# iesl/anncur

Measured on AMD Instinct MI355X. Metric: queries/sec + Top-k-Recall@100 vs exact, CUR-256 on QxI score matrix, higher is better.
Workload: dtype bf16; 1 GPU; cfg2: Q=10000/GPU x I=100000 bf16 score matrix, 256 anchor items, 512 anchor queries, k=100, k_retvr=100; step = gather C_q + fused S_hat/top-k + exact top-k scan + overlap/recall; Q_per_gpu=10000, I=100000, anchors=256, anchor_queries=512, k=100, k_retvr=100

## Files before the change

### anncur_amd/csrc/score16.hpp

```cpp
#pragma once

typedef __attribute__((ext_vector_type(4))) float f32x4;

template <int KP, int NW = 4>
struct Fused16Cfg {
	static constexpr int WAVES = NW;
	static constexpr int KS32 = KP / 32;
	static constexpr int K = KP / 16;
	static constexpr int CPR = KP / 8;
	static constexpr int TILE_BYTES = TILE_I * KP * 2;
	static constexpr int QCAP = 1024;
	static constexpr int DRAIN_AT = 192;
	static constexpr int QUEUE_OFF = 2 * TILE_BYTES;
	static constexpr int CNT_OFF = QUEUE_OFF + NW * QCAP * 8;
	static constexpr int TICKET_OFF = CNT_OFF + NW * 64 * 4;
	static constexpr int PIECES = TILE_BYTES / 1024 / NW;
	static_assert(PIECES >= 1, "a tile holds at least one 1 KB piece per wave");
	static constexpr int LVL_OFF = TICKET_OFF + 16;
	static constexpr int LCNT_OFF = LVL_OFF + NW * 64 * 4 * LADDER_LEVELS;
	static constexpr int JCUR_OFF = LCNT_OFF + NW * 64 * 16;
	static constexpr int LDS_BYTES = JCUR_OFF + NW * 64 * 4;
	static_assert(NW != 4 || LDS_BYTES <= 80 * 1024, "two workgroups per CU");
	static_assert(LADDER_LEVELS == 8, "two 128-bit reads per query; eight 16-bit fields in four counter words");
	static constexpr int BQ = 64 * NW;
};
#ifndef ANNCUR_LADDER_PERIOD
#define ANNCUR_LADDER_PERIOD 16
#endif
constexpr int LADDER_PERIOD = ANNCUR_LADDER_PERIOD;
constexpr uint32_t WQ_ITEM_BITS = 26, WQ_ITEM_MASK = (1u << WQ_ITEM_BITS) - 1u;

struct WaveQueue {
	uint32_t base, limit;
	uint32_t cnt;
	uint2 *seg;
	uint32_t q_stride8;
	uint32_t capg, n_items;
	int lane;
	uint32_t lad_on, lvl, jcur;
	uint32_t *lcnt;
};

template <bool LAD = false>
__device__ __forceinline__ void wq_drain(const WaveQueue &w, uint32_t &fill) {
	const uint32_t n = (fill - w.base) >> 3;
	unsigned char *const segb = reinterpret_cast<unsigned char *>(w.seg);
#pragma nounroll
	for (uint32_t i0 = 0; i0 < n; i0 += 64) {
		const uint32_t i = i0 + (uint32_t)w.lane;
		if (i < n) {
			const uint2 e = lds_load_u64(w.base + i * 8u);
			const uint32_t item = e.y & WQ_ITEM_MASK, ql = e.y >> WQ_ITEM_BITS;
			if (item < w.n_items) {
				uint32_t pos = 0;
#if defined(__HIP_DEVICE_COMPILE__)
				const uint32_t one = 1u;
				asm volatile("ds_add_rtn_u32 %0, %1, %2\n\ts_waitcnt lgkmcnt(0)" : "=&v"(pos) : "v"(w.cnt + ql * 4u), "v"(one) : "memory");
#endif
				if (pos < w.capg) *reinterpret_cast<uint2 *>(segb + (ql * w.q_stride8 + pos * 8u)) = make_uint2(e.x, item);
				if (LAD && w.lad_on) {
					f32x4 la = {0.f, 0.f, 0.f, 0.f}, lb = {0.f, 0.f, 0.f, 0.f};
					uint32_t jc = 0;
#if defined(__HIP_DEVICE_COMPILE__)
					asm volatile("ds_read_b128 %0, %3\n\tds_read_b128 %1, %3 offset:16\n\tds_read_b32 %2, %4\n\ts_waitcnt lgkmcnt(0)"
								 : "=&v"(la), "=&v"(lb), "=&v"(jc) : "v"(w.lvl + ql * 32u), "v"(w.jcur + ql * 4u) : "memory");
#endif
					const float v = __uint_as_float(e.x);
					const uint32_t j = (uint32_t)(v >= la[0]) + (uint32_t)(v >= la[1]) + (uint32_t)(v >= la[2]) + (uint32_t)(v >= la[3])
									   + (uint32_t)(v >= lb[0]) + (uint32_t)(v >= lb[1]) + (uint32_t)(v >= lb[2]) + (uint32_t)(v >= lb[3]);
					if (j > jc)
						(void)__hip_atomic_fetch_add(w.lcnt + ql * 4u + ((j - 1u) >> 1), 1u << (16u * ((j - 1u) & 1u)), __ATOMIC_RELAXED, __HIP_MEMORY_SCOPE_AGENT);
				}
			}
		}
	}
	fill = w.base;
}

__device__ __forceinline__ void filter16_one(float v, uint32_t code, float tau, uint32_t item0c, const WaveQueue &w, uint32_t &fill) {
	const bool hit = v >= tau;
	const unsigned long long m = __ballot(hit);
	if (__builtin_expect(m != 0ull, 0)) {
		if (hit) {
			const uint32_t rank = __builtin_amdgcn_mbcnt_hi((uint32_t)(m >> 32), __builtin_amdgcn_mbcnt_lo((uint32_t)m, 0u));
			lds_write_2x32(fill + rank * 8u, __float_as_uint(v), item0c + code);
		}
		fill += 8u * (uint32_t)__builtin_popcountll(m);
	}
}

__device__ __forceinline__ uint32_t opaque_u32(uint32_t x) {
#if defined(__HIP_DEVICE_COMPILE__)
	asm volatile("" : "+v"(x));
#endif
	return x;
}
__device__ __forceinline__ void ladder_fetch(const uint32_t *lcnt_wave, uint32_t land, int lane) {
#if defined(__HIP_DEVICE_COMPILE__)
	const uint32_t voff = (uint32_t)lane * 16u;
	asm volatile("s_mov_b32 m0, %0\n\ts_nop 0\n\tglobal_load_lds_dwordx4 %1, %2 sc1" ::"s"(land), "v"(voff), "s"(lcnt_wave) : "memory", "m0");
#endif
}

__device__ __forceinline__ void ladder_refresh(uint32_t lcnt_lane, uint32_t lvl_lane, uint32_t jcur_lane, uint32_t k, int c16, float (&tau)[4]) {
	u32x4 c = {0u, 0u, 0u, 0u};
	f32x4 la = {0.f, 0.f, 0.f, 0.f}, lb = {0.f, 0.f, 0.f, 0.f};
	uint32_t jc = 0;
#if defined(__HIP_DEVICE_COMPILE__)
	asm volatile("ds_read_b128 %0, %4\n\tds_read_b128 %1, %5\n\tds_read_b128 %2, %5 offset:16\n\tds_read_b32 %3, %6\n\ts_waitcnt lgkmcnt(0)"
				 : "=&v"(c), "=&v"(la), "=&v"(lb), "=&v"(jc) : "v"(lcnt_lane), "v"(lvl_lane), "v"(jcur_lane) : "memory");
#endif
	const float lv[8] = {la[0], la[1], la[2], la[3], lb[0], lb[1], lb[2], lb[3]};
	uint32_t cum = 0, jn = 0;
	float tn = -INFINITY;
#pragma unroll
	for (int j = 8; j >= 1; --j) {
		cum += (c[(j - 1) >> 1] >> (16 * ((j - 1) & 1))) & 0xffffu;
		const bool take = jn == 0u && cum >= k;
		jn = take ? (uint32_t)j : jn;
		tn = take ? lv[j - 1] : tn;
	}
	if (jn > jc) lds_write_u32(jcur_lane, jn);
#pragma unroll
	for (int t = 0; t < 4; ++t) {
		const float o = __int_as_float(__builtin_amdgcn_ds_bpermute((16 * t + c16) * 4, __float_as_int(tn)));
		tau[t] = fmaxf(tau[t], o);
	}
}

template <int KP, int CUR>
__device__ __forceinline__ void stagger16_tile(const uint32_t (&aoff)[Fused16Cfg<KP>::K], const bf16x8 (&xb)[4][Fused16Cfg<KP>::KS32], f32x4 (&accP)[2][2],
												const float (&tau)[4], const float (&tau_prev)[2], uint32_t item0, uint32_t item0_prev, const WaveQueue &w,
												uint32_t &fill) {
	using C = Fused16Cfg<KP>;
	constexpr int K = C::K, AR = 5, DIST = 3, OFF = CUR * C::TILE_BYTES;
	constexpr int EPS = 16 / K > 0 ? 16 / K : 1;
	static_assert(K <= 16 && 2 * K >= DIST, "staggered path: 4..16 steps per half");
	u32x4 ring[AR];
#pragma unroll
	for (int i = 0; i < DIST; ++i) lds_read_frag<OFF>(ring[i], aoff[i % K]);
	f32x4 accA[2][2], accB[2][2];
#pragma unroll
	for (int ih = 0; ih < 2; ++ih)
#pragma unroll
		for (int q = 0; q < 2; ++q) { accA[ih][q] = (f32x4){0.f, 0.f, 0.f, 0.f}; accB[ih][q] = (f32x4){0.f, 0.f, 0.f, 0.f}; }
#define F16_ELEM(ACC, e, QS0, TAU, ITEM0)                                                                                       \
	filter16_one(ACC[(e) >> 3][((e) >> 2) & 1][(e) & 3],                                                                        \
				 (uint32_t)((((e) >> 3) * 16 + ((e) & 3)) | ((uint32_t)((QS0) + (((e) >> 2) & 1)) << (WQ_ITEM_BITS + 4))),     \
				 TAU[((e) >> 2) & 1], ITEM0, w, fill)
#pragma unroll
	for (int g = 0; g < 2 * K; ++g) {
		const int nxt = g + DIST;
		if (nxt < 2 * K) lds_read_frag<OFF>(ring[nxt % AR], aoff[nxt % K]);
#if defined(__HIP_DEVICE_COMPILE__)
		if (g >= 1) asm volatile("" ::"v"(ring[(g - 1) % AR]));
#endif
		if (g > 0 && (g * EPS) % 8 == 0 && __builtin_expect(fill > w.limit, 0)) wq_drain<false>(w, fill);
		const int after = 2 * K - 1 - g;
		lds_wait_frag(ring[g % AR], after < DIST ? after : DIST);
		const bf16x8 a = __builtin_bit_cast(bf16x8, ring[g % AR]);
		const int s = g % K, ks = s >> 1, ih = s & 1;
		if (g < K) {
			accA[ih][0] = __builtin_amdgcn_mfma_f32_16x16x32_bf16(a, xb[0][ks], accA[ih][0], 0, 0, 0);
			accA[ih][1] = __builtin_amdgcn_mfma_f32_16x16x32_bf16(a, xb[1][ks], accA[ih][1], 0, 0, 0);
#pragma unroll
			for (int e = (g == 1 ? 0 : g) * EPS; e < (g == 0 ? 0 : g + 1) * EPS; ++e) F16_ELEM(accP, e, 2, tau_prev, item0_prev);
		} else {
			accB[ih][0] = __builtin_amdgcn_mfma_f32_16x16x32_bf16(a, xb[2][ks], accB[ih][0], 0, 0, 0);
			accB[ih][1] = __builtin_amdgcn_mfma_f32_16x16x32_bf16(a, xb[3][ks], accB[ih][1], 0, 0, 0);
#pragma unroll
			for (int e = (g - K == 1 ? 0 : g - K) * EPS; e < (g == K ? 0 : g - K + 1) * EPS; ++e) F16_ELEM(accA, e, 0, tau, item0);
		}
	}
#pragma unroll
	for (int ih = 0; ih < 2; ++ih)
#pragma unroll
		for (int q = 0; q < 2; ++q) accP[ih][q] = accB[ih][q];
}

#define S16_SLICED (p.sliced)
template <int KP, int NW = 4>
__global__ __launch_bounds__(64 * NW, 2) void score16_kernel(const FusedParams p) {
	using C = Fused16Cfg<KP, NW>;
	constexpr int K = C::K, KS32 = C::KS32, CPR = C::CPR;
	extern __shared__ __attribute__((aligned(16))) unsigned char smem[];
	const int tid = threadIdx.x, lane = tid & 63, wave = tid >> 6;
	const int c16 = lane & 15, g4 = lane >> 4;
	const int wid = xcd_remap(blockIdx.x, p.n_wg);
	const int n_rb = (int)((p.Q + C::BQ - 1) / C::BQ);
	const int split = p.rb_major ? wid % p.S : wid / n_rb, rb = p.rb_major ? wid / p.S : wid - split * n_rb;

	bf16x8 xb[4][KS32];
	int64_t qv[4];
#pragma unroll
	for (int t = 0; t < 4; ++t) {
		qv[t] = (int64_t)rb * C::BQ + wave * 64 + 16 * t + c16;
		const bool ok = qv[t] < p.Q;
		const u32x4 *src = reinterpret_cast<const u32x4 *>(p.X + (ok ? qv[t] : 0) * p.ldx) + g4;
#pragma unroll
		for (int s = 0; s < KS32; ++s) {
			const u32x4 zero = {0u, 0u, 0u, 0u};
			const u32x4 w = ok ? src[4 * s] : zero;
			xb[t][s] = __builtin_bit_cast(bf16x8, w);
		}
	}
	__builtin_amdgcn_s_waitcnt(0x0F70);

	const int j_begin = p.tile_begin + split * p.tiles_per_split, j_end = min(j_begin + p.tiles_per_split, p.tile_end);
	float tau[4];
#pragma unroll
	for (int t = 0; t < 4; ++t) tau[t] = qv[t] < p.Q ? p.tau[qv[t] * p.tau_stride] + p.tau_bias : INFINITY;
	const int wave_u = __builtin_amdgcn_readfirstlane(wave);
	const uint32_t lds_base = (uint32_t)__builtin_amdgcn_readfirstlane((int)lds_addr(smem));
	const int64_t q_wave0 = (int64_t)rb * C::BQ + wave_u * 64;
	WaveQueue w;
	w.base = lds_base + (uint32_t)(C::QUEUE_OFF + wave_u * C::QCAP * 8);
	w.limit = w.base + (uint32_t)(C::QCAP - 64 * (8 + 2 * (16 / K > 0 ? 16 / K : 1))) * 8u;
	w.cnt = lds_base + (uint32_t)(C::CNT_OFF + wave_u * 256);
	w.q_stride8 = (uint32_t)p.nseg * (uint32_t)p.capg * 8u;
	w.seg = p.cand + (q_wave0 * p.nseg + split) * (int64_t)p.capg;
	w.capg = (uint32_t)p.capg; w.n_items = (uint32_t)p.I; w.lane = lane;
	w.lad_on = (uint32_t)p.ladder_on;
	w.lvl = lds_base + (uint32_t)(C::LVL_OFF + wave_u * 64 * 4 * LADDER_LEVELS);
	w.jcur = lds_base + (uint32_t)(C::JCUR_OFF + wave_u * 256);
	w.lcnt = p.ladder_cnt + q_wave0 * 4;
	const uint32_t lcnt_land = lds_base + (uint32_t)(C::LCNT_OFF + wave_u * 1024);
	uint32_t fill = w.base;
	{
		const int64_t q = q_wave0 + lane;
		lds_write_u32(w.cnt + (uint32_t)lane * 4u, (p.carry && q < p.Q) ? p.seg_cnt[q * p.nseg + split] : 0u);
		lds_write_u32(w.jcur + (uint32_t)lane * 4u, 0u);
	}
	if (p.ladder_on) {
#if defined(__HIP_DEVICE_COMPILE__)
		const unsigned char *lsrc = reinterpret_cast<const unsigned char *>(p.ladder + q_wave0 * LADDER_LEVELS);
#pragma unroll
		for (int i = 0; i < 2; ++i) {
			const uint32_t m0v = w.lvl + (uint32_t)i * 1024u, voff = (uint32_t)(i * 1024 + lane * 16);
			asm volatile("s_mov_b32 m0, %0\n\ts_nop 0\n\tglobal_load_lds_dwordx4 %1, %2" ::"s"(m0v), "v"(voff), "s"(lsrc) : "memory", "m0");
		}
#endif
	}
	uint32_t lad_tick = 0;
	bool lad_pending = false;

	int t_cur = j_begin < j_end ? j_begin : -1, t_cend = j_end, t_next_chunk = -1;
	bool ticket_pending = false;
	const bool dyn = p.chunk_tiles > 0;
	uint32_t ticket_slot = lds_addr(smem + C::TICKET_OFF);
	uint32_t *const ctr_rb = p.chunk_ctr + (S16_SLICED ? (size_t)rb * N_SLICES : (size_t)rb);
	int slice = S16_SLICED ? xcc_id() : 0, tried = 0;
	if (dyn) {
		if (tid == 0) {
			uint32_t c0, c1;
			if (S16_SLICED) {
				c0 = slice_resolve(atomicAdd(ctr_rb + slice, 1u), ctr_rb, p.n_chunks, p.chunks_per_slice, slice, tried);
				c1 = c0 < (uint32_t)p.n_chunks ? slice_resolve(atomicAdd(ctr_rb + slice, 1u), ctr_rb, p.n_chunks, p.chunks_per_slice, slice, tried) : (uint32_t)p.n_chunks;
			} else {
				c0 = atomicAdd(ctr_rb, 2u); c1 = c0 + 1u;
			}
			if (p.chunk_owner) {
				if (c0 < (uint32_t)p.n_chunks) p.chunk_owner[(int64_t)rb * p.n_chunks + c0] = (uint8_t)split;
				if (c1 < (uint32_t)p.n_chunks) p.chunk_owner[(int64_t)rb * p.n_chunks + c1] = (uint8_t)split;
			}
			lds_write_u32(ticket_slot + 8u, c0);
			lds_write_u32(ticket_slot + 12u, c1);
			__builtin_amdgcn_s_waitcnt(0xC07F);
		}
		__syncthreads();
		const uint32_t c = lds_load_u32_uniform(ticket_slot + 8u), c1 = lds_load_u32_uniform(ticket_slot + 12u);
		t_cur = c < (uint32_t)p.n_chunks ? p.tile_begin + (int)c * p.chunk_tiles : -1;
		t_cend = min(t_cur + p.chunk_tiles, p.tile_end);
		t_next_chunk = c1 < (uint32_t)p.n_chunks ? p.tile_begin + (int)c1 * p.chunk_tiles : -1;
	}
	uint32_t dma_off[C::PIECES];
#pragma unroll
	for (int i = 0; i < C::PIECES; ++i) {
		const int pch = (wave_u * C::PIECES + i) * 64 + lane;
		const int row = pch / CPR, cs = pch % CPR;
		dma_off[i] = (uint32_t)(row * CPR + swz<CPR>(row, cs)) * 16u;
	}
	auto tile_dma_w = [&](int tile, uint32_t lds_buf) {
		const unsigned char *src = reinterpret_cast<const unsigned char *>(p.Et) + (int64_t)tile * C::TILE_BYTES;
#if defined(__HIP_DEVICE_COMPILE__)
#pragma unroll
		for (int i = 0; i < C::PIECES; ++i) {
			const uint32_t m0v = lds_buf + (uint32_t)(wave_u * C::PIECES + i) * 1024u;
			asm volatile("s_mov_b32 m0, %0\n\ts_nop 0\n\tglobal_load_lds_dwordx4 %1, %2" ::"s"(m0v), "v"(dma_off[i]), "s"(src) : "memory", "m0");
		}
#endif
	};
	if (t_cur >= 0) tile_dma_w(t_cur, lds_base);
	__builtin_amdgcn_s_waitcnt(0x0F70);
	__syncthreads();

	f32x4 accP[2][2];
#pragma unroll
	for (int ih = 0; ih < 2; ++ih)
#pragma unroll
		for (int q = 0; q < 2; ++q) accP[ih][q] = (f32x4){0.f, 0.f, 0.f, 0.f};
	float tau_prev[2] = {INFINITY, INFINITY};
	uint32_t item0_prev = 0;
	uint32_t aoff[K];
#pragma unroll
	for (int s = 0; s < K; ++s) {
		const int row = 16 * (s & 1) + c16;
		aoff[s] = lds_addr(smem) + (uint32_t)(row * CPR + swz<CPR>(row, 4 * (s >> 1) + g4)) * 16u;
	}
	const uint32_t lane_code = (uint32_t)c16 << WQ_ITEM_BITS;
	__builtin_amdgcn_s_waitcnt(0xC07F);
	float tau_hi[2] = {tau[2], tau[3]};
#define R16_DRAIN_CHECK(J) do { if (fill >= w.base + C::DRAIN_AT * 8u) wq_drain<true>(w, fill); } while (0)
#define LADDER_STEP()                                                                                                           \
	do {                                                                                                                        \
		if (p.ladder_on) {                                                                                                      \
			const uint32_t ll_ = opaque_u32((uint32_t)lane);    \
			if (lad_pending) {                                                                                                  \
				ladder_refresh(lcnt_land + ll_ * 16u, w.lvl + ll_ * 32u, w.jcur + ll_ * 4u, p.ladder_k, (int)(ll_ & 15u), tau);     \
				tau_hi[0] = tau[2]; tau_hi[1] = tau[3];                                                                         \
				tau_prev[0] = fmaxf(tau_prev[0], tau[2]); tau_prev[1] = fmaxf(tau_prev[1], tau[3]);                             \
				lad_pending = false;                                                                                            \
			}                                                                                                                   \
			if ((++lad_tick & p.ladder_mask) == 0u) {                                                                           \
				ladder_fetch(w.lcnt, lcnt_land, (int)ll_);                                                                      \
				lad_pending = true;                                                                                             \
			}                                                                                                                   \
		}                                                                                                                       \
	} while (0)
#define STAGGER16_STEP(CUR)                                                                                                     \
	do {                                                                                                                        \
		const int J = t_cur;                                                                                                    \
		if (ticket_pending) {                                                                                                   \
			const uint32_t c = lds_load_u32_uniform(ticket_slot);                                                               \
			t_next_chunk = c < (uint32_t)p.n_chunks ? p.tile_begin + (int)c * p.chunk_tiles : -1;                               \
			ticket_pending = false;                                                                                             \
			ticket_slot ^= 4u;                                                                                                  \
		}                                                                                                                       \
		int nx = J + 1;                                                                                                         \
		bool crossed = false;                                                                                                   \
		if (nx >= t_cend) { nx = t_next_chunk; crossed = dyn && nx >= 0; }                                                      \
		if (nx >= 0) tile_dma_w(nx, lds_base + ((CUR) ^ 1) * C::TILE_BYTES);                                                    \
		uint32_t ticket = 0;                                                                                                    \
		if (crossed && tid == 0) ticket_draw(ticket, ctr_rb + slice);                                                           \
		LADDER_STEP();                                                                                                          \
		R16_DRAIN_CHECK(J);                                                                                                     \
		const uint32_t item0 = ((uint32_t)J * TILE_I + 4 * g4) | lane_code;                                                     \
		stagger16_tile<KP, CUR>(aoff, xb, accP, tau, tau_prev, item0, item0_prev, w, fill);                                        \
		tau_prev[0] = tau_hi[0]; tau_prev[1] = tau_hi[1]; item0_prev = item0;                                                   \
		ticket_wait(ticket);                                                                                                    \
		if (crossed) {                                                                                                          \
			if (tid == 0) {                                                                                                     \
				if (S16_SLICED) ticket = slice_resolve(ticket, ctr_rb, p.n_chunks, p.chunks_per_slice, slice, tried);             \
				lds_write_u32(ticket_slot, ticket);                                                                             \
				if (p.chunk_owner && ticket < (uint32_t)p.n_chunks) p.chunk_owner[(int64_t)rb * p.n_chunks + ticket] = (uint8_t)split; \
				__builtin_amdgcn_s_waitcnt(0xC07F);                                                                             \
			}                                                                                                                   \
			ticket_pending = true;                                                                                              \
			t_cend = min(nx + p.chunk_tiles, p.tile_end);                                                                       \
		}                                                                                                                       \
		__syncthreads();                                                                                                        \
		t_cur = nx;                                                                                                             \
	} while (0)
	ANNCUR_PAD_HERE();
	while (t_cur >= 0) {
		STAGGER16_STEP(0);
		if (t_cur < 0) break;
		STAGGER16_STEP(1);
	}
#undef STAGGER16_STEP
#undef LADDER_STEP
	wq_drain<true>(w, fill);
#define F16_LAST(e)                                                                                                             \
	filter16_one(accP[(e) >> 3][((e) >> 2) & 1][(e) & 3],                                                                       \
				 (uint32_t)((((e) >> 3) * 16 + ((e) & 3)) | ((uint32_t)(2 + (((e) >> 2) & 1)) << (WQ_ITEM_BITS + 4))),         \
				 tau_prev[((e) >> 2) & 1], item0_prev, w, fill)
	F16_LAST(0); F16_LAST(1); F16_LAST(2); F16_LAST(3); F16_LAST(4); F16_LAST(5); F16_LAST(6); F16_LAST(7);
	F16_LAST(8); F16_LAST(9); F16_LAST(10); F16_LAST(11); F16_LAST(12); F16_LAST(13); F16_LAST(14); F16_LAST(15);
#undef F16_LAST
#undef F16_ELEM
	wq_drain<true>(w, fill);
	if (p.ladder_on) {
		const int le = (int)opaque_u32((uint32_t)lane);
		__builtin_amdgcn_s_waitcnt(0x0F70);
		ladder_fetch(w.lcnt, lcnt_land, le);
		__builtin_amdgcn_s_waitcnt(0x0F70);
		ladder_refresh(lcnt_land + (uint32_t)le * 16u, w.lvl + (uint32_t)le * 32u, w.jcur + (uint32_t)le * 4u, p.ladder_k, le & 15, tau);
		if ((le >> 4) == 0) {
#pragma unroll
			for (int t = 0; t < 4; ++t) {
				const int64_t qe = q_wave0 + 16 * t + (le & 15);
				if (qe < p.Q) {
					if (tau[t] >= 0.f) atomicMax(reinterpret_cast<int *>(p.tau_final + qe), __float_as_int(tau[t]));
					else atomicMin(reinterpret_cast<unsigned int *>(p.tau_final + qe), __float_as_uint(tau[t]));
				}
			}
		}
	}
	{
		const int64_t q = q_wave0 + lane;
		uint32_t c = 0;
#if defined(__HIP_DEVICE_COMPILE__)
		asm volatile("ds_read_b32 %0, %1\n\ts_waitcnt lgkmcnt(0)" : "=&v"(c) : "v"(w.cnt + (uint32_t)lane * 4u) : "memory");
#endif
		if (q < p.Q) p.seg_cnt[q * p.nseg + split] = c;
	}
}
```

### anncur_amd/csrc/score_fused.hip

```cpp
#include <stdlib.h>
#include <math.h>
#include <type_traits>
#ifdef ANNCUR_PLACEMENT_PAD
#define ANNCUR_PAD_HERE() asm volatile(".rept %0\n\ts_nop 0\n\t.endr" ::"n"(ANNCUR_PLACEMENT_PAD) : "memory")
#else
#define ANNCUR_PAD_HERE() do { } while (0)
#endif
#include "select.hpp"
#include "wave_select.hpp"
#include "select_stream.hpp"

using namespace anncur;

namespace {

typedef __attribute__((ext_vector_type(8))) __bf16 bf16x8;
typedef __attribute__((ext_vector_type(16))) float f32x16;
typedef __attribute__((ext_vector_type(4))) unsigned int u32x4;

constexpr int TILE_I = 32;
constexpr int CHUNK_TILES = 4;

template <int KP, int QTV = ((KP <= 256) ? 2 : 1)>
struct FusedCfg {
// ... 1175 lines not shown
		if (!TAU_ONLY && lane == 0) hard_list[atomicAdd(hard_cnt, 1u)] = (int32_t)q;
		return;
	}
	constexpr int CAP = WqCfg<KW>::CAP, TRIGGER = WqCfg<KW>::TRIGGER;
	WaveSel w = wsel_init<CAP>(smem + wave * WaveSelLayout<CAP>::BYTES);
	if (tau && prefilter) w.tau = tau[q * tau_stride];
	const uint2 *qc = cand + q * nseg * (int64_t)capg;
	constexpr int LOAD_U = 8;
	for (uint32_t j0 = 0; j0 < total; j0 += LOAD_U * WAVE) {
		int sg[LOAD_U];
#pragma unroll
		for (int u = 0; u < LOAD_U; ++u) sg[u] = 0;
#pragma unroll
		for (int step = 32; step >= 1; step >>= 1) {
			if (step < nseg) {
				uint32_t pv[LOAD_U];
#pragma unroll
				for (int u = 0; u < LOAD_U; ++u) pv[u] = __shfl(pre, (sg[u] + step) & 63);
#pragma unroll
				for (int u = 0; u < LOAD_U; ++u)
					if (sg[u] + step < nseg && pv[u] <= j0 + (uint32_t)(u * WAVE + lane)) sg[u] += step;
			}
		}
		uint32_t ps[LOAD_U];
#pragma unroll
		for (int u = 0; u < LOAD_U; ++u) ps[u] = __shfl(pre, sg[u]);
		uint2 e[LOAD_U];
#pragma unroll
		for (int u = 0; u < LOAD_U; ++u) {
			const uint32_t j = j0 + (uint32_t)(u * WAVE + lane);
			e[u] = qc[j < total ? (int64_t)sg[u] * capg + (j - ps[u]) : 0];
		}
#pragma unroll
		for (int u = 0; u < LOAD_U; ++u) {
			if (j0 + (uint32_t)(u * WAVE) < total) {
				wsel_offer(w, j0 + (uint32_t)(u * WAVE + lane) < total, __uint_as_float(e[u].x), e[u].y);
				if (w.cnt > (uint32_t)TRIGGER) wsel_compact<4, false, true>(w, k);
			}
		}
	}
	if (TAU_ONLY) {
		if (w.cnt > k) wsel_compact<4, false, true>(w, k);
		if (lane == 0 && w.cnt >= k) tau[q * tau_stride] = fmaxf(tau[q * tau_stride], w.tau);
		return;
	}
	wsel_finish<0, 4, WqCfg<KW>::E, true>(w, k, out_val + q * (int64_t)k, out_idx + q * (int64_t)k, remap);
}

}
namespace {
#include "score_wide.hpp"
}
namespace {

struct FusedPlan {
	bool ok;
	int QT, BQ, n_rb, n_tiles, n_full, S, tiles_per_split, group, n_st, S0, st_per_split, n_groups, capg, kmax, flush_tiles;
	int n_stages, stage_end[3], stage_tps[3], stage_flush[3], stage_pred[3];
	int leading;
	int lg;
	bool body16;
	bool bodyef;
	bool bodyq16;
	int chunk;
	bool ladder;
	int ladder_k2;
	size_t off_lcnt, off_lvl, off_tau2;
	size_t off_gmax, off_tval, off_tidx, off_segcnt, off_cand, off_tau, off_hard, off_ctr, off_owner, total;
};

int num_cu() { return anncur_num_cu(); }

size_t align256(size_t x) { return (x + 255) & ~(size_t)255; }
int next_pow2(int x) { int p = 1; while (p < x) p <<= 1; return p; }

void plan_stages(FusedPlan &P, int64_t Q, int k, double exp_hits, bool staged, double fmin, int unit_items) {
	double frac[3] = {1.0, 1.0, 1.0};
	P.n_stages = 1;
	if (staged) {
		const double H0 = exp_hits, c_hit = 2.4e-11 * (double)Q;
		const double c_stage = k <= WSEL_K ? 25e-6 + 3e-9 * (double)Q : (k <= WQ_K2 ? 25e-6 + 1.2e-8 * (double)Q : 25e-6 + 1.4e-11 * (double)Q * 0.3 * H0);
		auto later = [&](double f) { const double h = 1.2 * k / f; return h < H0 ? h : H0; };
		double best = H0 * c_hit;
		static const double grid[] = {0.02, 0.03, 0.04, 0.06, 0.08, 0.10, 0.12, 0.15, 0.18, 0.22, 0.26, 0.30, 0.35, 0.40, 0.50};
		const int ng = (int)(sizeof(grid) / sizeof(grid[0]));
		for (int i = 0; i < ng; ++i) {
			const double f1 = grid[i];
			if (f1 < fmin) continue;
			const double c2 = (f1 * H0 + (1 - f1) * later(f1)) * c_hit + c_stage;
			if (c2 < best) { best = c2; P.n_stages = 2; frac[0] = f1; frac[1] = 1.0; }
			for (int j = i + 1; j < ng; ++j) {
				const double f2 = grid[j];
				if (f2 - f1 < fmin) continue;
				const double c3 = (f1 * H0 + (f2 - f1) * later(f1) + (1 - f2) * later(f2)) * c_hit + 2 * c_stage;
				if (c3 < best) { best = c3; P.n_stages = 3; frac[0] = f1; frac[1] = f2; }
			}
		}
	}
	if (P.n_stages == 2) {
		const double shrink = P.body16 ? 0.63 : (k <= WSEL_K ? 1.0 : 0.6);
		const double f1 = frac[0] * shrink;
		frac[0] = f1 > fmin ? f1 : (fmin < frac[0] ? fmin : frac[0]);
	}
	double rate = exp_hits / ((double)P.n_tiles * 2.0);
	int prev = 0;
	for (int i = 0; i < P.n_stages; ++i) {
		int end = (int)(frac[i] * P.n_tiles + 0.5);
		if (i == P.n_stages - 1 || end > P.n_tiles) end = P.n_tiles;
		if (end <= prev) end = prev + 1 < P.n_tiles ? prev + 1 : P.n_tiles;
		P.stage_end[i] = end;
		P.stage_tps[i] = (end - prev + P.S - 1) / P.S;
		int ft = (int)(0.35 / (rate > 1e-9 ? rate : 1e-9));
		P.stage_flush[i] = ft < 1 ? 1 : (ft > 8 ? 8 : ft);
		P.stage_pred[i] = (1.0 - exp(-4.0 * rate)) > 0.25 ? 1 : 0;
		rate = (double)k / ((double)end * unit_items) * 16.0 * 1.2;
		prev = end;
	}
}

FusedPlan plan_fused(int64_t Q, int64_t I, int KP, int k, bool leading = false, bool mfma16 = false, bool qt1 = false, bool mfma32 = false, bool evalf = false,
					 bool no_ladder = false) {
	FusedPlan P{};
	P.ok = false;
	P.leading = leading ? 1 : 0;
	if (!(KP == 64 || KP == 128 || KP == 256 || KP == 512)) return P;
	if (k < 1 || k > ANNCUR_MAX_TOPK || Q < 1 || I < 1 || I >= (int64_t)0x7fffffff - 64 || k > I) return P;
	if (evalf && !(KP <= 256 && I < (int64_t)(1 << 26))) return P;
	if (evalf) { qt1 = false; mfma16 = false; mfma32 = false; leading = false; P.leading = 0; }
	P.bodyef = evalf;
	P.QT = (KP <= 256 && !(qt1 && KP >= 128)) ? 2 : 1;
	P.BQ = 128 * P.QT;
	P.n_rb = (int)ceil_div64(Q, P.BQ);
	P.n_tiles = (int)ceil_div64(I, TILE_I);
	P.n_full = (int)(I / TILE_I);
	int target = (4 * k > 512) ? 4 * k : 512;
	int n_st16 = (target + 1) / 2;
	if ((int64_t)n_st16 * 8 <= P.n_full) { P.group = 16; P.n_st = n_st16; }
	else { P.group = 4; P.n_st = (target + 7) / 8; }
	if ((int64_t)P.n_st * 4 > P.n_full) return P;
	P.n_groups = P.n_st * (P.group == 16 ? 2 : 8);
	if (P.n_groups < k) return P;
	int slots = ((P.QT == 1 && KP <= 256) ? 3 : 2) * num_cu();
	P.bodyq16 = KP == 512 && !mfma32 && I < (int64_t)(1 << 26);
	const bool ticketed = (P.QT == 2 || P.bodyq16) && !evalf;
	P.chunk = ticketed ? CHUNK_TILES : 0;
	const bool can16 = KP <= 256 && P.QT == 2 && I < (int64_t)(1 << 26);
	constexpr int BODY16_MAX_K = 384, BODY16_MAX_K_LADDER = 1024;
	const bool ladder_possible = !no_ladder && ticketed && P.n_groups <= 4096;
	P.body16 = can16 && !mfma32 && !evalf && (mfma16 || k <= (ladder_possible ? BODY16_MAX_K_LADDER : BODY16_MAX_K));
	int S = P.chunk > 0 ? (slots + P.n_rb - 1) / P.n_rb : slots / P.n_rb;
	if (P.chunk > 0 && k <= WQ_K2 && S > WAVE / 2) S = WAVE / 2;
	if (S < 1) S = 1;
	if (S > 255) S = P.chunk > 0 ? 255 : (S > 256 ? 256 : S);
	if (S > P.n_tiles) S = P.n_tiles;
	P.tiles_per_split = (P.n_tiles + S - 1) / S;
	P.S = (P.n_tiles + P.tiles_per_split - 1) / P.tiles_per_split;
	int S0 = slots / P.n_rb;
	if (S0 < 1) S0 = 1;
	if (S0 > P.n_st) S0 = P.n_st;
	P.st_per_split = (P.n_st + S0 - 1) / S0;
	P.S0 = (P.n_st + P.st_per_split - 1) / P.st_per_split;
	P.lg = (P.body16 || P.bodyq16 || P.bodyef) ? 1 : 2;
	const double exp_hits_cap = 1.3 * k * ((double)P.n_tiles / P.n_st);
	const double exp_hits = (leading ? 0.65 : 1.0) * exp_hits_cap;
	const double per_seg = exp_hits_cap / ((double)P.lg * P.S);
	int capg = next_pow2((int)(4.0 * per_seg) + 32);
	if (capg < 64) capg = 64;
	if (capg > 16384) capg = 16384;
	P.capg = capg;
	const double per_lane_tile = exp_hits / ((double)P.n_tiles * 2.0);
	int ft = (int)(0.35 / (per_lane_tile > 1e-9 ? per_lane_tile : 1e-9));
	P.flush_tiles = ft < 1 ? 1 : (ft > 8 ? 8 : ft);
	P.ladder = P.body16 && !no_ladder && P.n_groups <= 4096 && P.chunk > 0;
	{
		double r = (double)k * ((double)P.n_st * TILE_I / (double)I) * (leading ? 2.0 : 1.25);
		int k2 = (int)(r + 0.5);
		if (k2 > k / 2) k2 = k / 2;
		if (k2 < 3) k2 = 3;
		if (k2 > k) k2 = k;
		P.ladder_k2 = k2;
	}
	plan_stages(P, Q, k, exp_hits, !P.ladder && (k <= WQ_K2 ? P.lg * P.S <= WAVE : true) && P.n_tiles >= 24 * P.S, 4.0 * P.S / P.n_tiles, TILE_I);
	P.kmax = k <= 128 ? 128 : (k <= 512 ? 512 : 2048);
	size_t off = 256;
	P.off_ctr = off;    off = align256(off + (size_t)P.n_rb * 3 * 4 * N_SLICES);
	P.off_lcnt = off;   off = align256(off + (P.ladder ? (size_t)P.n_rb * P.BQ * 16 : 0));
	P.off_gmax = off;   off = align256(off + (size_t)Q * P.n_groups * 4);
	P.off_tval = off;   off = align256(off + (size_t)Q * k * 4);
	P.off_tidx = off;   off = align256(off + (size_t)Q * k * 4);
	P.off_segcnt = off; off = align256(off + (size_t)Q * P.lg * P.S * 4);
	P.off_tau = off;    off = align256(off + (size_t)Q * 4);
	P.off_hard = off;   off = align256(off + (size_t)Q * 4);
	P.off_owner = off;  off = align256(off + (size_t)3 * P.n_rb * (size_t)(P.n_tiles / (P.chunk > 0 ? P.chunk : P.n_tiles) + 2));
	P.off_lvl = off;    off = align256(off + (P.ladder ? (size_t)P.n_rb * P.BQ * 4 * LADDER_LEVELS : 0));
	P.off_tau2 = off;   off = align256(off + (P.ladder ? (size_t)Q * 4 : 0));
	P.off_cand = off;   off = align256(off + (size_t)Q * P.lg * P.S * (size_t)P.capg * 8);
	P.total = off;
	P.ok = true;
	return P;
}

#define EV(i) do { if (ev) ANNCUR_HIP_OK(hipEventRecord(ev[i], st)); } while (0)

constexpr bool STREAM_SELECT_SMALL = false;

int launch_tau_refine(const uint2 *cand, const uint32_t *seg_cnt, int nseg, int capg, int64_t Q, int k, int kmax, float *tau, int tau_stride,
					  int prefilter, hipStream_t st) {
	int rc;
	if (k <= WQ_K2 && nseg <= WAVE) {
#define LAUNCH_WTAU(KW)                                                                                                           \
		do {                                                                                                                      \
			constexpr int lds = 4 * WaveSelLayout<WqCfg<KW>::CAP>::BYTES;                                                         \
			if ((rc = anncur_ensure_dyn_lds((const void *)select_wave_kernel<true, KW>, lds)) != ANNCUR_OK) return rc;            \
			hipLaunchKernelGGL((select_wave_kernel<true, KW>), dim3((unsigned)ceil_div64(Q, 4)), dim3(256), lds, st, cand, seg_cnt, nseg, capg, Q, \
							   (uint32_t)k, (float *)nullptr, (int32_t *)nullptr, (uint32_t *)nullptr, (int32_t *)nullptr, tau, tau_stride, prefilter, (const int32_t *)nullptr); \
		} while (0)
		if (k <= WSEL_K) LAUNCH_WTAU(128);
		else {
			constexpr int lds = 4 * StreamSelLayout::BYTES;
			hipLaunchKernelGGL((select_stream_kernel<true, 2>), dim3((unsigned)ceil_div64(Q, 4)), dim3(256), lds, st, cand, seg_cnt, nseg, capg, Q,
							   (uint32_t)k, (float *)nullptr, (int32_t *)nullptr, (uint32_t *)nullptr, (int32_t *)nullptr, tau, tau_stride, prefilter, (const int32_t *)nullptr);
		}
#undef LAUNCH_WTAU
	} else {
#define LAUNCH_TAU(KM)                                                                                                        \
		do {                                                                                                                  \
			if ((rc = anncur_ensure_dyn_lds((const void *)tau_block_kernel<KM>, (int)SelCfg<KM>::LDS_BYTES)) != ANNCUR_OK) return rc; \
			hipLaunchKernelGGL((tau_block_kernel<KM>), dim3((unsigned)Q), dim3(SEL_THREADS), SelCfg<KM>::LDS_BYTES, st, cand, seg_cnt, \
							   nseg, capg, (uint32_t)k, tau, tau_stride, prefilter);                                           \
		} while (0)
		if (kmax == 128) LAUNCH_TAU(128); else if (kmax == 512) LAUNCH_TAU(512); else LAUNCH_TAU(2048);
#undef LAUNCH_TAU
	}
	ANNCUR_LAUNCH_OK();
	return ANNCUR_OK;
}

int launch_select(const FusedPlan &P, int nseg, const SweepStages &stages, const uint2 *cand, const uint32_t *seg_cnt, const uint16_t *X, int64_t ldx,
				  const uint16_t *Et, int64_t Q, int64_t I, int KP, int k, float *out_val, int32_t *out_idx, unsigned char *ws, const float *tau,
				  int tau_stride, hipStream_t st, const int32_t *remap = nullptr) {
	int rc;
#define LAUNCH_SELECT(KM)                                                                                              \
	do {                                                                                                               \
		const size_t lds = SelCfg<KM>::LDS_BYTES + (size_t)KP * 4 + 32;                                                \
		if ((rc = anncur_ensure_dyn_lds((const void *)select_candidates_kernel<KM>, (int)lds)) != ANNCUR_OK) return rc; \
		hipLaunchKernelGGL((select_candidates_kernel<KM>), dim3(sel_grid), dim3(SEL_THREADS), lds, st, cand, seg_cnt, nseg, \
						   P.S, stages, P.capg, X, ldx, Et, I, KP, (uint32_t)k, out_val, out_idx, (uint32_t *)ws, hard_list, hard_cnt,      \
						   (P.n_stages > 1 || P.ladder) ? tau : (const float *)nullptr, tau_stride, remap);                              \
	} while (0)
	const int32_t *hard_list = nullptr;
	const uint32_t *hard_cnt = nullptr;
	unsigned sel_grid = (unsigned)Q;
	if (k <= WQ_K2 && nseg <= WAVE) {
		int32_t *hl = (int32_t *)(ws + P.off_hard);
		uint32_t *hc = (uint32_t *)(ws + 4);
#define LAUNCH_WSEL(KW)                                                                                                           \
		do {                                                                                                                      \
			constexpr int lds = 4 * WaveSelLayout<WqCfg<KW>::CAP>::BYTES;                                                         \
			if ((rc = anncur_ensure_dyn_lds((const void *)select_wave_kernel<false, KW>, lds)) != ANNCUR_OK) return rc;           \
			hipLaunchKernelGGL((select_wave_kernel<false, KW>), dim3((unsigned)ceil_div64(Q, 4)), dim3(256), lds, st, cand, seg_cnt, nseg, P.capg, Q, \
							   (uint32_t)k, out_val, out_idx, hc, hl, const_cast<float *>(tau), tau_stride, (P.n_stages > 1 || P.ladder) ? 1 : 0, remap); \
		} while (0)
#define LAUNCH_SSEL(EE)                                                                                                           \
		do {                                                                                                                      \
			constexpr int lds = 4 * StreamSelLayout::BYTES;                                                                       \
			hipLaunchKernelGGL((select_stream_kernel<false, EE>), dim3((unsigned)ceil_div64(Q, 4)), dim3(256), lds, st, cand, seg_cnt, nseg, P.capg, Q, \
							   (uint32_t)k, out_val, out_idx, hc, hl, const_cast<float *>(tau), tau_stride, (P.n_stages > 1 || P.ladder) ? 1 : 0, remap); \
		} while (0)
		if (k <= WSEL_K) { if (STREAM_SELECT_SMALL) LAUNCH_SSEL(2); else LAUNCH_WSEL(128); }
		else if (k <= 256) LAUNCH_SSEL(4);
		else if (k <= 512) LAUNCH_SSEL(8);
		else LAUNCH_SSEL(16);
#undef LAUNCH_SSEL
#undef LAUNCH_WSEL
		ANNCUR_LAUNCH_OK();
		hard_list = hl; hard_cnt = hc;
		sel_grid = (unsigned)(Q < 1024 ? Q : 1024);
	}
	if (P.kmax == 128) LAUNCH_SELECT(128); else if (P.kmax == 512) LAUNCH_SELECT(512); else LAUNCH_SELECT(2048);
#undef LAUNCH_SELECT
	ANNCUR_LAUNCH_OK();
	return ANNCUR_OK;
}

int launch_threshold(const FusedPlan &P, const float *gmax, int64_t Q, int k, unsigned char *ws, const float *&tau, int &tau_stride, hipStream_t st) {
	if (P.n_groups <= 4096) {
		float *t = (float *)(ws + P.off_tau);
		const int rc = P.ladder ? anncur_internal_kth_value(gmax, Q, P.n_groups, P.n_groups, k, t, 1, st, 1, (float *)(ws + P.off_lvl), P.ladder_k2, (float *)(ws + P.off_tau2))
								: anncur_internal_kth_value(gmax, Q, P.n_groups, P.n_groups, k, t, 1, st, 1);
		tau = t; tau_stride = 1;
		return rc;
	}
	float *tval = (float *)(ws + P.off_tval);
	tau = tval + (k - 1); tau_stride = k;
	return anncur_rowwise_topk(gmax, ANNCUR_F32, Q, P.n_groups, P.n_groups, k, tval, (int32_t *)(ws + P.off_tidx), st);
}


struct CoScan {
	hipStream_t aux;
	hipEvent_t *ev;
	const void *A; int a_dtype; int64_t lda, Q, I; int32_t k;
	float *val; int32_t *idx;
	int slots, next;
	int64_t row_end[8];
};
// ... 554 lines not shown
```

Measured before the change: 11.52 million queries/s.

## Restructure body16 tile loop into single sweep with interleaved DMA and filter

Replaces the staggered two-half tile routine with a single sweep that computes all four query sub-tiles per A-fragment read. It ping-pongs two accumulator sets so the previous tile's filter runs inside the current tile's MFMA steps, and it issues the next tile's global-to-LDS DMA pieces within the first steps instead of before the tile. It also changes the LDS fragment addressing to fewer precomputed offsets. The intent is fewer LDS fragment reads per tile and better overlap of DMA, MFMA and filtering, at the cost of more accumulator registers and a larger pending filter backlog at the end.

```diff
diff --git a/anncur_amd/csrc/score16.hpp b/anncur_amd/csrc/score16.hpp
--- a/anncur_amd/csrc/score16.hpp
+++ b/anncur_amd/csrc/score16.hpp
@@ -8,6 +8,7 @@
 	static constexpr int KS32 = KP / 32;
 	static constexpr int K = KP / 16;
 	static constexpr int CPR = KP / 8;
+	static constexpr int NA = KS32 < 4 ? KS32 : 4;
 	static constexpr int TILE_BYTES = TILE_I * KP * 2;
 	static constexpr int QCAP = 1024;
 	static constexpr int DRAIN_AT = 192;
@@ -128,54 +129,52 @@
 	}
 }
 
+__device__ __forceinline__ void tile_dma_piece(const unsigned char *src, uint32_t m0v, uint32_t voff) {
+#if defined(__HIP_DEVICE_COMPILE__)
+	asm volatile("s_mov_b32 m0, %0\n\ts_nop 0\n\tglobal_load_lds_dwordx4 %1, %2" ::"s"(m0v), "v"(voff), "s"(src) : "memory", "m0");
+#endif
+}
+
+#define F16_ELEM(ACC, e, TAU, ITEM0)                                                                                            \
+	filter16_one(ACC[(e) >> 4][((e) >> 2) & 3][(e) & 3],                                                                        \
+				 (uint32_t)((((e) >> 4) * 16 + ((e) & 3)) | ((uint32_t)(((e) >> 2) & 3) << (WQ_ITEM_BITS + 4))), TAU[((e) >> 2) & 3], ITEM0, w, fill)
+
 template <int KP, int CUR>
-__device__ __forceinline__ void stagger16_tile(const uint32_t (&aoff)[Fused16Cfg<KP>::K], const bf16x8 (&xb)[4][Fused16Cfg<KP>::KS32], f32x4 (&accP)[2][2],
-												const float (&tau)[4], const float (&tau_prev)[2], uint32_t item0, uint32_t item0_prev, const WaveQueue &w,
-												uint32_t &fill) {
+__device__ __forceinline__ void sweep16_tile(const uint32_t (&aoff)[Fused16Cfg<KP>::NA], const bf16x8 (&xb)[4][Fused16Cfg<KP>::KS32], f32x4 (&acc)[2][4],
+											 const f32x4 (&accP)[2][4], const float (&tau)[4], uint32_t item0_prev, const WaveQueue &w, uint32_t &fill,
+											 const unsigned char *dma_src, uint32_t dma_m0, const uint32_t (&dma_off)[Fused16Cfg<KP>::PIECES]) {
 	using C = Fused16Cfg<KP>;
-	constexpr int K = C::K, AR = 5, DIST = 3, OFF = CUR * C::TILE_BYTES;
-	constexpr int EPS = 16 / K > 0 ? 16 / K : 1;
-	static_assert(K <= 16 && 2 * K >= DIST, "staggered path: 4..16 steps per half");
+	constexpr int K = C::K, NA = C::NA, AR = 4, DIST = 2, OFF = CUR * C::TILE_BYTES;
+	constexpr int EPS = 32 / K;
+	static_assert(C::PIECES <= K / 2, "the DMA pieces go out in the first half of the steps");
+	static_assert(K >= 4 && K <= 16 && K >= DIST, "4..16 steps per tile");
+#define S16_READ(slot, s) lds_read_frag_at(ring[slot], aoff[((s) >> 1) % NA], OFF + ((s) & 1) * 16 * C::CPR * 16 + (((s) >> 1) / NA) * 256)
 	u32x4 ring[AR];
 #pragma unroll
-	for (int i = 0; i < DIST; ++i) lds_read_frag<OFF>(ring[i], aoff[i % K]);
-	f32x4 accA[2][2], accB[2][2];
+	for (int i = 0; i < DIST; ++i) S16_READ(i, i);
 #pragma unroll
 	for (int ih = 0; ih < 2; ++ih)
 #pragma unroll
-		for (int q = 0; q < 2; ++q) { accA[ih][q] = (f32x4){0.f, 0.f, 0.f, 0.f}; accB[ih][q] = (f32x4){0.f, 0.f, 0.f, 0.f}; }
-#define F16_ELEM(ACC, e, QS0, TAU, ITEM0)                                                                                       \
-	filter16_one(ACC[(e) >> 3][((e) >> 2) & 1][(e) & 3],                                                                        \
-				 (uint32_t)((((e) >> 3) * 16 + ((e) & 3)) | ((uint32_t)((QS0) + (((e) >> 2) & 1)) << (WQ_ITEM_BITS + 4))),     \
-				 TAU[((e) >> 2) & 1], ITEM0, w, fill)
-#pragma unroll
-	for (int g = 0; g < 2 * K; ++g) {
+		for (int t = 0; t < 4; ++t) acc[ih][t] = (f32x4){0.f, 0.f, 0.f, 0.f};
+#pragma unroll
+	for (int g = 0; g < K; ++g) {
 		const int nxt = g + DIST;
-		if (nxt < 2 * K) lds_read_frag<OFF>(ring[nxt % AR], aoff[nxt % K]);
+		if (nxt < K) S16_READ(nxt % AR, nxt);
 #if defined(__HIP_DEVICE_COMPILE__)
 		if (g >= 1) asm volatile("" ::"v"(ring[(g - 1) % AR]));
 #endif
 		if (g > 0 && (g * EPS) % 8 == 0 && __builtin_expect(fill > w.limit, 0)) wq_drain<false>(w, fill);
-		const int after = 2 * K - 1 - g;
+		const int after = K - 1 - g;
 		lds_wait_frag(ring[g % AR], after < DIST ? after : DIST);
 		const bf16x8 a = __builtin_bit_cast(bf16x8, ring[g % AR]);
-		const int s = g % K, ks = s >> 1, ih = s & 1;
-		if (g < K) {
-			accA[ih][0] = __builtin_amdgcn_mfma_f32_16x16x32_bf16(a, xb[0][ks], accA[ih][0], 0, 0, 0);
-			accA[ih][1] = __builtin_amdgcn_mfma_f32_16x16x32_bf16(a, xb[1][ks], accA[ih][1], 0, 0, 0);
-#pragma unroll
-			for (int e = (g == 1 ? 0 : g) * EPS; e < (g == 0 ? 0 : g + 1) * EPS; ++e) F16_ELEM(accP, e, 2, tau_prev, item0_prev);
-		} else {
-			accB[ih][0] = __builtin_amdgcn_mfma_f32_16x16x32_bf16(a, xb[2][ks], accB[ih][0], 0, 0, 0);
-			accB[ih][1] = __builtin_amdgcn_mfma_f32_16x16x32_bf16(a, xb[3][ks], accB[ih][1], 0, 0, 0);
-#pragma unroll
-			for (int e = (g - K == 1 ? 0 : g - K) * EPS; e < (g == K ? 0 : g - K + 1) * EPS; ++e) F16_ELEM(accA, e, 0, tau, item0);
-		}
-	}
-#pragma unroll
-	for (int ih = 0; ih < 2; ++ih)
-#pragma unroll
-		for (int q = 0; q < 2; ++q) accP[ih][q] = accB[ih][q];
+		const int ks = g >> 1, ih = g & 1;
+#pragma unroll
+		for (int t = 0; t < 4; ++t) acc[ih][t] = __builtin_amdgcn_mfma_f32_16x16x32_bf16(a, xb[t][ks], acc[ih][t], 0, 0, 0);
+		if (g < C::PIECES) tile_dma_piece(dma_src, dma_m0 + (uint32_t)g * 1024u, dma_off[g]);
+#pragma unroll
+		for (int e = g * EPS; e < (g + 1) * EPS; ++e) F16_ELEM(accP, e, tau, item0_prev);
+	}
+#undef S16_READ
 }
 
 #define S16_SLICED (p.sliced)
@@ -215,7 +214,7 @@
 	const int64_t q_wave0 = (int64_t)rb * C::BQ + wave_u * 64;
 	WaveQueue w;
 	w.base = lds_base + (uint32_t)(C::QUEUE_OFF + wave_u * C::QCAP * 8);
-	w.limit = w.base + (uint32_t)(C::QCAP - 64 * (8 + 2 * (16 / K > 0 ? 16 / K : 1))) * 8u;
+	w.limit = w.base + (uint32_t)(C::QCAP - 64 * 8) * 8u;
 	w.cnt = lds_base + (uint32_t)(C::CNT_OFF + wave_u * 256);
 	w.q_stride8 = (uint32_t)p.nseg * (uint32_t)p.capg * 8u;
 	w.seg = p.cand + (q_wave0 * p.nseg + split) * (int64_t)p.capg;
@@ -294,22 +293,17 @@
 	__builtin_amdgcn_s_waitcnt(0x0F70);
 	__syncthreads();
 
-	f32x4 accP[2][2];
+	f32x4 acc0[2][4], acc1[2][4];
 #pragma unroll
 	for (int ih = 0; ih < 2; ++ih)
 #pragma unroll
-		for (int q = 0; q < 2; ++q) accP[ih][q] = (f32x4){0.f, 0.f, 0.f, 0.f};
-	float tau_prev[2] = {INFINITY, INFINITY};
+		for (int t = 0; t < 4; ++t) { acc0[ih][t] = (f32x4){NAN, NAN, NAN, NAN}; acc1[ih][t] = acc0[ih][t]; }
 	uint32_t item0_prev = 0;
-	uint32_t aoff[K];
-#pragma unroll
-	for (int s = 0; s < K; ++s) {
-		const int row = 16 * (s & 1) + c16;
-		aoff[s] = lds_addr(smem) + (uint32_t)(row * CPR + swz<CPR>(row, 4 * (s >> 1) + g4)) * 16u;
-	}
+	uint32_t aoff[C::NA];
+#pragma unroll
+	for (int s = 0; s < C::NA; ++s) aoff[s] = lds_addr(smem) + (uint32_t)(c16 * CPR + swz<CPR>(c16, 4 * s + g4)) * 16u;
 	const uint32_t lane_code = (uint32_t)c16 << WQ_ITEM_BITS;
 	__builtin_amdgcn_s_waitcnt(0xC07F);
-	float tau_hi[2] = {tau[2], tau[3]};
 #define R16_DRAIN_CHECK(J) do { if (fill >= w.base + C::DRAIN_AT * 8u) wq_drain<true>(w, fill); } while (0)
 #define LADDER_STEP()                                                                                                           \
 	do {                                                                                                                        \
@@ -317,8 +311,6 @@
 			const uint32_t ll_ = opaque_u32((uint32_t)lane);    \
 			if (lad_pending) {                                                                                                  \
 				ladder_refresh(lcnt_land + ll_ * 16u, w.lvl + ll_ * 32u, w.jcur + ll_ * 4u, p.ladder_k, (int)(ll_ & 15u), tau);     \
-				tau_hi[0] = tau[2]; tau_hi[1] = tau[3];                                                                         \
-				tau_prev[0] = fmaxf(tau_prev[0], tau[2]); tau_prev[1] = fmaxf(tau_prev[1], tau[3]);                             \
 				lad_pending = false;                                                                                            \
 			}                                                                                                                   \
 			if ((++lad_tick & p.ladder_mask) == 0u) {                                                                           \
@@ -339,14 +331,16 @@
 		int nx = J + 1;                                                                                                         \
 		bool crossed = false;                                                                                                   \
 		if (nx >= t_cend) { nx = t_next_chunk; crossed = dyn && nx >= 0; }                                                      \
-		if (nx >= 0) tile_dma_w(nx, lds_base + ((CUR) ^ 1) * C::TILE_BYTES);                                                    \
+		 \
+		const unsigned char *dsrc = reinterpret_cast<const unsigned char *>(p.Et) + (int64_t)(nx >= 0 ? nx : J) * C::TILE_BYTES;     \
 		uint32_t ticket = 0;                                                                                                    \
 		if (crossed && tid == 0) ticket_draw(ticket, ctr_rb + slice);                                                           \
 		LADDER_STEP();                                                                                                          \
 		R16_DRAIN_CHECK(J);                                                                                                     \
 		const uint32_t item0 = ((uint32_t)J * TILE_I + 4 * g4) | lane_code;                                                     \
-		stagger16_tile<KP, CUR>(aoff, xb, accP, tau, tau_prev, item0, item0_prev, w, fill);                                        \
-		tau_prev[0] = tau_hi[0]; tau_prev[1] = tau_hi[1]; item0_prev = item0;                                                   \
+		sweep16_tile<KP, CUR>(aoff, xb, (CUR) ? acc1 : acc0, (CUR) ? acc0 : acc1, tau, item0_prev, w, fill, dsrc,                \
+							  lds_base + ((CUR) ^ 1) * C::TILE_BYTES + (uint32_t)(wave_u * C::PIECES) * 1024u, dma_off);              \
+		item0_prev = item0;                                                                                                     \
 		ticket_wait(ticket);                                                                                                    \
 		if (crossed) {                                                                                                          \
 			if (tid == 0) {                                                                                                     \
@@ -364,19 +358,23 @@
 	ANNCUR_PAD_HERE();
 	while (t_cur >= 0) {
 		STAGGER16_STEP(0);
-		if (t_cur < 0) break;
+		if (t_cur < 0) {
+#pragma unroll
+			for (int ih = 0; ih < 2; ++ih)
+#pragma unroll
+				for (int t = 0; t < 4; ++t) acc1[ih][t] = acc0[ih][t];
+			break;
+		}
 		STAGGER16_STEP(1);
 	}
 #undef STAGGER16_STEP
 #undef LADDER_STEP
 	wq_drain<true>(w, fill);
-#define F16_LAST(e)                                                                                                             \
-	filter16_one(accP[(e) >> 3][((e) >> 2) & 1][(e) & 3],                                                                       \
-				 (uint32_t)((((e) >> 3) * 16 + ((e) & 3)) | ((uint32_t)(2 + (((e) >> 2) & 1)) << (WQ_ITEM_BITS + 4))),         \
-				 tau_prev[((e) >> 2) & 1], item0_prev, w, fill)
-	F16_LAST(0); F16_LAST(1); F16_LAST(2); F16_LAST(3); F16_LAST(4); F16_LAST(5); F16_LAST(6); F16_LAST(7);
-	F16_LAST(8); F16_LAST(9); F16_LAST(10); F16_LAST(11); F16_LAST(12); F16_LAST(13); F16_LAST(14); F16_LAST(15);
-#undef F16_LAST
+#pragma unroll
+	for (int e = 0; e < 16; ++e) F16_ELEM(acc1, e, tau, item0_prev);
+	wq_drain<true>(w, fill);
+#pragma unroll
+	for (int e = 16; e < 32; ++e) F16_ELEM(acc1, e, tau, item0_prev);
 #undef F16_ELEM
 	wq_drain<true>(w, fill);
 	if (p.ladder_on) {
diff --git a/anncur_amd/csrc/score_fused.hip b/anncur_amd/csrc/score_fused.hip
--- a/anncur_amd/csrc/score_fused.hip
+++ b/anncur_amd/csrc/score_fused.hip
@@ -1351,6 +1351,7 @@
 	if (P.chunk > 0 && k <= WQ_K2 && S > WAVE / 2) S = WAVE / 2;
 	if (S < 1) S = 1;
 	if (S > 255) S = P.chunk > 0 ? 255 : (S > 256 ? 256 : S);
+	static_assert(WQ_K2 + (WAVE / 2) * (LADDER_PERIOD + 2) * TILE_I < 65536, "ladder counter fields: S x (LADDER_PERIOD + 2) x 32 + k < 2^16");
 	if (S > P.n_tiles) S = P.n_tiles;
 	P.tiles_per_split = (P.n_tiles + S - 1) / S;
 	P.S = (P.n_tiles + P.tiles_per_split - 1) / P.tiles_per_split;
```

Measured after the change: 11.63 million queries/s (median of 6 runs). No clear change (+0.9%).
